# vpc-ccg/freddie

Hardware: AMD Instinct MI355X
Metric: reads segmented/sec (whole node) (higher is better)
Workload: dtype u32

## Files before the change

### freddie_amd/csrc/freddie_seg.hip

```cpp
#include "seg_kernels.h"

using namespace fseg;

namespace {

struct DevBuf {
    void *p = nullptr;
    size_t cap = 0;
    template <typename T> T *as() const { return reinterpret_cast<T *>(p); }
};
struct Slab {
    void *p = nullptr;
    size_t cap = 0;
};
struct HostBuf {
    void *p = nullptr;
    size_t cap = 0;
    template <typename T> T *as() const { return reinterpret_cast<T *>(p); }
};
struct Carve {
    struct Item { DevBuf *b; size_t off, bytes; };
    std::vector<Item> items;
    size_t total = 0;
    size_t add(DevBuf &b, size_t bytes) {
// ... 55 lines not shown
    DevBuf d_packed;
    int fetched_packed = -1;
    bool label_packed_ok = true;
    bool label_has2 = false;
    bool run_label_packed = false;
    bool labels_unpacked = false;
    DevBuf d_sort_tmp;
    DevBuf d_part_iv_off, d_part_rep_off, d_part_lane_off, d_iv_start, d_iv_end, d_pos_off, d_iv_part,
        d_rep_exon_off, d_rep_weight, d_ex_ts, d_ex_te, d_tile_desc, d_iv_tile0, d_blk_iv0, d_rb_part, d_rb_r0, d_rb_sum, d_rb_base, d_rb_max, d_rb_cmax,
        d_hc_part, d_hc_p0, d_hc_n, d_hc_glo, d_hc_ghi;
    DevBuf d_lane_ex, d_lane_start, d_lane_pmax, d_hc_llo, d_hc_lhi, d_key_a, d_key_b, d_val_a, d_val_b, d_rep_last;
    DevBuf d_lane_lx, d_lex, d_rb_esum, d_rb_ebase;
    i64 max_rep_exons = 0;
    DevBuf d_w_main, d_w_refine, d_h_table, d_thr_tab;
    DevBuf d_bits;
    DevBuf d_y_raw, d_y, d_v, d_scan_state, d_bsum, d_bsum_side, d_g, d_pk, d_pf, d_kp;
    int n_hist_chunks = 0;
    DevBuf d_voff, d_chunk_off, d_csum, d_mean, d_thr, d_label_off, d_part_has2;
    int n_rep_blocks = 0;
    DevBuf d_cand_off, d_cand_y, d_fixed0, d_added, d_fixed, d_chosen, d_final_off, d_final_y, d_final_pos, d_final_iv, d_col_thr,
        d_col_zero;
    DevBuf d_tile_defer;
    DevBuf d_blk_pre, d_tile_tot, d_seg_iv, d_seg_prev, d_rseg_c, d_cand_pn, d_cand_ll, d_cand_ln, d_cand_wide, d_prob_bs;
    DevBuf d_prob_iv, d_prob_start, d_prob_n, d_prob_pair_off, d_prob_tri_off, d_prob_flags, d_prob_chain,
        d_prob_cov_off, d_prob_lane_lo, d_prob_lane_n;
    DevBuf d_dp_items, d_solve_items, d_solve_desc, d_prob_desc, d_work_pc, d_cls_items, d_work_active, d_pair_thr, d_amb, d_out, d_cov;
    DevBuf d_wide_items;
    DevBuf d_wide_all;
    DevBuf d_dpx;
    i64 dpx_base[3] = {0, 0, 0}, dpx_stride[3] = {0, 0, 0}, dpx_n[3] = {0, 0, 0};
    int dpx_nm = 0, dpx_cnt[3] = {1, 1, 1};
// ... 298 lines not shown
        if (!dev_sync) return;
        for (int k = 1; k < ps.n_seg; ++k) if (dev_side(k)) (void)fork(ps.side_of[k]);
    };
    auto launch_fork_waiters = [&]() {
        if (!dev_sync) return;
        for (int k = 1; k < ps.n_seg; ++k) if (dev_side(k))
            hipLaunchKernelGGL(k_wait_word, dim3(1), dim3(64), 0, c->side[ps.side_of[k]], st, &sw->emit_gen, 1u, sync_gen, kSyncTicks);
    };
    const i64 avg_len = NPOS / (K > 0 ? K : 1);
    const int iv_threads = avg_len > 65536 ? 1024 : (avg_len > 16384 ? 256 : 64);
    int tile_grid = grid_for(c->n_tiles, 1, 16384);
    const i64 scan_nb = scan_blocks(NPOS);
    const int scan_grid = scan_nb > 0 ? (int)scan_nb : 1;
    u64 *scan_state = c->d_scan_state.as<u64>();
    const bool scan_single = scan_nb <= c->scan_single_max;
    int *bsum = scan_single ? nullptr : c->d_bsum.as<int>();
    int *bsum_side = scan_single ? nullptr : c->d_bsum_side.as<int>();
    auto scan_counts = [&](hipStream_t q, int *bs, const unsigned *flags, u64 *total_dev, i64 *off_last) {
        if (scan_single) return;
        hipLaunchKernelGGL(k_scan1, dim3(grid_for(scan_nb, 1, 4096)), dim3(256), 0, q, flags, NPOS, bs);
        hipLaunchKernelGGL(k_scan2, dim3(1), dim3(kScan2Threads), 0, q, bs, scan_nb, total_dev, off_last);
    };
    int work_grid = grid_for(c->work_cap, 1, 4096);
    ProblemArrays pr{c->d_prob_iv.as<int>(), c->d_prob_start.as<int>(), c->d_prob_n.as<int>(),
                     c->d_prob_pair_off.as<i64>(), c->d_prob_tri_off.as<i64>(), c->d_prob_flags.as<int>(),
                     c->d_prob_chain.as<int>(), c->d_prob_cov_off.as<i64>(), c->d_prob_lane_lo.as<int>(),
                     c->d_prob_lane_n.as<int>()};
    const int pg = grid_for(NPOS / 8 / kProbBlock + 1, 1, 1024);
    i64 *prob_bs = (c->prob_self_scan && !sized) ? nullptr : c->d_prob_bs.as<i64>();
    if (do_pre1) {
    {
        const i64 nw = 3 * (i64)flag_words(NPOS);
// ... 24 lines not shown
#undef FSEG_LAUNCH_SMOOTH
    end(ST_SMOOTH);
    {
    hipStream_t q = fork(0);
    if (stage_events && c->profile_all) (void)hipEventRecord(c->ev_b[ST_THRESHOLD], q);
    const bool thr_part_fits = c->max_part_pos <= (i64)kThrPartMaxChunks * 8192;
    const bool thr_part = thr_part_fits && (c->thr_part == 1 || (c->thr_part < 0 && n_part >= 64));
    if (thr_part) {
        c->paths[fseg_ctx::PATH_THR_PART] = 1;
        hipLaunchKernelGGL(k_thr_part, dim3(grid_for(n_part, 1, 4096)), dim3(512), 0, q, n_part, c->d_part_iv_off.as<i64>(), c->d_pos_off.as<i64>(), NPOS,
                           flag_pos_bits, c->d_y.as<double>(), c->d_v.as<double>(), c->P.variance_factor, c->d_mean.as<double>(), c->d_thr.as<double>());
    } else {
    c->paths[fseg_ctx::PATH_THR_PART] = 0;
    scan_counts(q, bsum_side, flag_pos_bits, &st->n_vals, nullptr);
    hipLaunchKernelGGL(k_scan_emit<kEmitValues>, dim3(scan_grid), dim3(256), 0, q, flag_pos_bits, NPOS,
                       bsum_side, scan_state, &st->n_vals, (i64 *)nullptr, &st->err, c->d_y.as<double>(), c->d_v.as<double>(), K, c->d_pos_off.as<i64>(),
                       c->d_iv_start.as<int>(), c->d_blk_iv0.as<int>(), (int *)nullptr, (int *)nullptr, (i64 *)nullptr,
                       c->force_scan_stall ? 1 : 0, (int *)nullptr);
    hipLaunchKernelGGL(k_voff, dim3(grid_for(n_part + 1, 1, 2048)), dim3(64), 0, q, n_part, c->d_part_iv_off.as<i64>(),
                       c->d_pos_off.as<i64>(), NPOS, flag_pos_bits, bsum_side, scan_state, &st->n_vals,
                       c->d_voff.as<i64>());
    hipLaunchKernelGGL(k_vplan, dim3(1), dim3(256), 0, q, n_part, c->d_part_iv_off.as<i64>(), c->d_pos_off.as<i64>(), NPOS,
                       c->d_voff.as<i64>(), c->d_chunk_off.as<i64>(), st, c->chunk_cap);
    int chunk_grid = grid_for(c->chunk_cap, 1, 4096);
    double *csum0 = c->d_csum.as<double>(), *csum1 = csum0 + c->chunk_cap;
    for (int pass = 0; pass < 2; ++pass)
        hipLaunchKernelGGL(k_vsum_chunks, dim3(chunk_grid), dim3(512), 0, q, n_part, c->d_voff.as<i64>(),
                           c->d_chunk_off.as<i64>(), c->d_v.as<double>(), csum0, pass, pass ? csum1 : csum0, c->chunk_cap);
    hipLaunchKernelGGL(k_vsum_part, dim3(grid_for(n_part, 64, 1024)), dim3(64), 0, q, n_part, c->d_voff.as<i64>(),
                       c->d_chunk_off.as<i64>(), csum0, csum1, c->P.variance_factor, c->d_mean.as<double>(),
                       c->d_thr.as<double>(), c->chunk_cap);
    }
    if (stage_events && c->profile_all) (void)hipEventRecord(c->ev_e[ST_THRESHOLD], q);
    }
    begin(ST_CANDIDATES);
    hipLaunchKernelGGL(k_peaks_edges, dim3(grid_for(c->n_tiles, 256, 4096)), dim3(256), 0, s, c->n_tiles, c->d_tile_desc.as<TileDesc>(),
                       c->d_tile_defer.as<int>(), c->d_y.as<double>(), flag_cand_bits, c->d_part_has2.as<int>(), n_part);
    scan_counts(s, bsum, flag_cand_bits, &st->n_cand, c->d_cand_off.as<i64>() + K);
    hipLaunchKernelGGL(k_scan_emit<kEmitPositions>, dim3(scan_grid), dim3(256), 0, s, flag_cand_bits, NPOS,
                       bsum, scan_state + scan_nb, &st->n_cand, c->d_cand_off.as<i64>() + K, &st->err, (const double *)nullptr, (double *)nullptr, K, c->d_pos_off.as<i64>(),
                       c->d_iv_start.as<int>(), c->d_blk_iv0.as<int>(), c->d_cand_y.as<int>(), (int *)nullptr,
                       c->d_cand_off.as<i64>(), 0, (int *)nullptr);
    end(ST_CANDIDATES);
    join(0);
    early_fork();
    begin(ST_FIX);
    c->paths[fseg_ctx::PATH_IV_THREADS] = iv_threads;
    hipLaunchKernelGGL(k_fix, dim3(grid_for(K, 1, 8192)), dim3(iv_threads), 0, s, K, c->d_pos_off.as<i64>(),
                       c->d_iv_part.as<int>(), c->d_cand_off.as<i64>(), c->d_cand_y.as<int>(), c->d_y.as<double>(),
                       c->d_thr.as<double>(), c->P.max_problem_size, c->d_fixed0.as<unsigned char>(),
                       c->d_added.as<unsigned char>(), c->d_fixed.as<unsigned char>(), c->d_chosen.as<unsigned char>(),
                       c->d_cand_pn.as<int>(), c->d_seg_iv.as<int>(), st);
    i64 *range_bs = prob_bs;
    hipLaunchKernelGGL(k_prob_range, dim3(pg), dim3(kRangeThreads), 0, s, st, c->d_cand_pn.as<int>(),
                       c->d_seg_iv.as<int>(), c->d_cand_y.as<int>(), c->d_iv_part.as<int>(), c->d_iv_start.as<int>(),
// ... 332 lines not shown
                               pr, c->d_prob_desc.as<ProbDesc>(), c->prob_cap, c->d_cand_y.as<int>(), c->d_out.as<unsigned>(),
                               c->tri_cap, c->d_amb.as<unsigned>(), c->d_pair_thr.as<int2>(), c->pair_cap,
                               c->P.min_read_support_outside, c->d_chosen.as<unsigned char>(), c->nm_giant,
                               c->d_giant.as<unsigned char>(), (i64)giant_scratch_bytes(c->nm_giant));
    }
    end(ST_DP); begin(ST_REFINE);
    hipLaunchKernelGGL(k_segments, dim3(grid_for(K, 1, 8192)), dim3(iv_threads), 0, s, K, c->d_pos_off.as<i64>(),
                       c->d_cand_off.as<i64>(), c->d_cand_y.as<int>(), c->d_y_raw.as<int>(), c->d_blk_pre.as<int>(), c->d_tile_tot.as<int>(), c->d_iv_tile0.as<int>(),
                       c->d_chosen.as<unsigned char>(), flag_final_bits, c->d_rseg_c.as<int>(),
                       c->d_seg_prev.as<int>(), st);
    hipLaunchKernelGGL(k_refine, dim3(2048), dim3(64), 0, s, st, c->d_seg_iv.as<int>(), c->d_rseg_c.as<int>(),
                       c->d_seg_prev.as<int>(), c->d_cand_y.as<int>(), c->d_pos_off.as<i64>(), c->d_y_raw.as<int>(),
                       c->d_w_refine.as<double>(), c->P.radius_refine, c->P.sigma, c->d_g.as<double>(), c->d_pk.as<int>(),
                       c->d_pf.as<unsigned char>(), c->d_kp.as<unsigned char>(), flag_final_bits);
    end(ST_REFINE); begin(ST_FINAL);
    scan_counts(s, bsum, flag_final_bits, &st->n_final, c->d_final_off.as<i64>() + K);
    hipLaunchKernelGGL(k_scan_emit<kEmitPositions>, dim3(scan_grid), dim3(256), 0, s, flag_final_bits,
                       NPOS, bsum, scan_state + 2 * scan_nb, &st->n_final, c->d_final_off.as<i64>() + K, &st->err, (const double *)nullptr, (double *)nullptr, K, c->d_pos_off.as<i64>(),
                       c->d_iv_start.as<int>(), c->d_blk_iv0.as<int>(), c->d_final_y.as<int>(), c->d_final_pos.as<int>(),
                       c->d_final_off.as<i64>(), 0, c->d_final_iv.as<int>());
    hipLaunchKernelGGL(k_label_cols, dim3(grid_for(NPOS / 8 + 1, 256, 2048)), dim3(256), 0, s, K, c->d_final_off.as<i64>(),
                       c->d_final_y.as<int>(), c->d_final_iv.as<int>(), c->d_iv_part.as<int>(), c->d_h_table.as<double>(), c->P.h_len,
                       c->P.threshold_rate, c->d_thr_tab.as<int2>(), c->d_col_thr.as<int2>(), c->d_col_zero.as<unsigned char>(),
                       c->d_part_has2.as<int>(), n_part, c->d_part_iv_off.as<i64>(), c->d_part_rep_off.as<i64>(),
                       c->d_label_off.as<i64>(), st, c->label_cap);
    end(ST_FINAL);
    }
    if (do_post2) {
    begin(ST_LABEL);
    if (c->label_cap > 0) {
        c->run_label_packed = lab_packed; c->labels_unpacked = false;
        c->paths[fseg_ctx::PATH_LABEL_PACKED] = lab_packed;
        if (lab_packed) {
// ... 551 lines not shown
        }
    }
    int hist_chunk = hist_packed ? kHistChunk16 : kHistChunk;
    while (hist_chunk > 1024 && NPOS / hist_chunk < 512) hist_chunk >>= 1;
    i64 n_chunks = 0;
    {
        i64 k = 0, pos = 0;
        for (int p = 0; p < np; ++p) {
            i64 Pp = 0;
            for (k = b->part_iv_off[p]; k < b->part_iv_off[p + 1]; ++k) Pp += (i64)b->iv_end[k] - b->iv_start[k] + 1;
            n_chunks += (Pp + hist_chunk - 1) / hist_chunk;
            pos += Pp;
        }
        (void)pos;
    }
    const i64 nb = scan_blocks(NPOS);
    if (n_tiles >= 0x7fffffffLL || n_chunks >= 0x7fffffffLL) return fail(c, FSEG_ERR_UNSUPPORTED, "batch too large");
    Carve in;
    in.add(c->d_part_iv_off, ((size_t)np + 1) * 8);
    in.add(c->d_part_rep_off, ((size_t)np + 1) * 8);
    in.add(c->d_part_lane_off, ((size_t)np + 1) * 8);
    in.add(c->d_iv_start, (size_t)K * 4);
    in.add(c->d_iv_end, (size_t)K * 4);
    in.add(c->d_pos_off, ((size_t)K + 1) * 8);
    in.add(c->d_iv_part, (size_t)K * 4);
    in.add(c->d_iv_tile0, (size_t)K * 4);
    in.add(c->d_tile_desc, (size_t)n_tiles * sizeof(TileDesc));
    in.add(c->d_blk_iv0, ((size_t)nb + 1) * 4);
    in.add(c->d_rb_part, (size_t)n_rep_blocks * 4);
    in.add(c->d_rb_r0, (size_t)n_rep_blocks * 4);
    in.add(c->d_hc_part, (size_t)n_chunks * 4);
    in.add(c->d_hc_p0, (size_t)n_chunks * 8);
    in.add(c->d_hc_n, (size_t)n_chunks * 4);
    in.add(c->d_hc_glo, (size_t)n_chunks * 4);
    in.add(c->d_hc_ghi, (size_t)n_chunks * 4);
    in.add(c->d_rep_exon_off, ((size_t)R + 1) * 8);
    in.add(c->d_rep_weight, (size_t)R * 4);
    in.add(c->d_ex_ts, (size_t)I * 4 + kExonPad);
    in.add(c->d_ex_te, (size_t)I * 4 + kExonPad);
    const size_t up_bytes = in.total;
    in.add(c->d_lane_ex, (size_t)lanes * 16);
    in.add(c->d_lane_start, (size_t)lanes * 4);
    in.add(c->d_lane_pmax, (size_t)lanes * 4);
// ... 25 lines not shown
        int *h_blk = reinterpret_cast<int *>(host_of(c->d_blk_iv0));
        int *h_rb_part = reinterpret_cast<int *>(host_of(c->d_rb_part)), *h_rb_r0 = reinterpret_cast<int *>(host_of(c->d_rb_r0));
        int *h_hc_part = reinterpret_cast<int *>(host_of(c->d_hc_part)), *h_hc_n = reinterpret_cast<int *>(host_of(c->d_hc_n));
        int *h_hc_glo = reinterpret_cast<int *>(host_of(c->d_hc_glo)), *h_hc_ghi = reinterpret_cast<int *>(host_of(c->d_hc_ghi));
        i64 *h_hc_p0 = reinterpret_cast<i64 *>(host_of(c->d_hc_p0));
        h_pos_off[0] = 0; h_lane_off[0] = 0; c->max_part_lanes = 0; c->max_part_pos = 0;
        i64 t = 0, rb = 0, ch = 0, l = 0, bq = 0;
        for (int p = 0; p < np; ++p) {
            const i64 k0 = b->part_iv_off[p], k1 = b->part_iv_off[p + 1];
            for (i64 k = k0; k < k1; ++k) {
                const i64 len = (i64)b->iv_end[k] - b->iv_start[k] + 1;
                h_iv_part[k] = p;
                h_pos_off[k + 1] = h_pos_off[k] + len;
                h_iv_tile0[k] = (int)t;
                for (i64 y = 0; y < len; y += kSmoothTile) h_tile[t++] = TileDesc{h_pos_off[k], (int)y, (int)len};
                for (; bq < nb && bq * kScanBlock < h_pos_off[k + 1]; ++bq) h_blk[bq] = (int)k;
            }
            for (i64 r = b->part_rep_off[p]; r < b->part_rep_off[p + 1]; r += 256) { h_rb_part[rb] = p; h_rb_r0[rb] = (int)r; ++rb; }
            for (i64 r = b->part_rep_off[p]; r < b->part_rep_off[p + 1]; ++r) l += b->rep_weight[r];
            h_lane_off[p + 1] = l;
            if (l - h_lane_off[p] > c->max_part_lanes) c->max_part_lanes = l - h_lane_off[p];
            const i64 P0 = h_pos_off[k0], P1 = h_pos_off[k1];
            if (P1 - P0 > c->max_part_pos) c->max_part_pos = P1 - P0;
            i64 k = k0;
            for (i64 q0 = P0; q0 < P1; q0 += hist_chunk) {
                const i64 q1 = std::min<i64>(q0 + hist_chunk, P1) - 1;
                while (h_pos_off[k + 1] <= q0) ++k;
                i64 kk = k;
                while (h_pos_off[kk + 1] <= q1) ++kk;
                h_hc_part[ch] = p; h_hc_p0[ch] = q0; h_hc_n[ch] = (int)(q1 - q0 + 1);
                h_hc_glo[ch] = b->iv_start[k] + (int)(q0 - h_pos_off[k]);
                h_hc_ghi[ch] = b->iv_start[kk] + (int)(q1 - h_pos_off[kk]);
                ++ch;
            }
        }
        h_blk[nb] = (int)(K - 1);
    }
    const double t_tables = tk.ms();
    memcpy(host_of(c->d_part_iv_off), b->part_iv_off, ((size_t)np + 1) * 8);
    memcpy(host_of(c->d_part_rep_off), b->part_rep_off, ((size_t)np + 1) * 8);
    memcpy(host_of(c->d_iv_start), b->iv_start, (size_t)K * 4);
    memcpy(host_of(c->d_iv_end), b->iv_end, (size_t)K * 4);
    memcpy(host_of(c->d_rep_exon_off), b->rep_exon_off, ((size_t)R + 1) * 8);
    memcpy(host_of(c->d_rep_weight), b->rep_weight, (size_t)R * 4);
    memcpy(host_of(c->d_ex_ts), b->ex_ts, (size_t)I * 4);
    memcpy(host_of(c->d_ex_te), b->ex_te, (size_t)I * 4);
    const double t_copy = tk.ms();
    c->n_part = np; c->K = K; c->R = R; c->I = I; c->NPOS = NPOS; c->LANES = lanes; c->expanded = expanded;
    if (c->max_part_lanes > lanes) c->max_part_lanes = lanes;
    c->n_tiles = (int)n_tiles; c->n_hist_chunks = (int)n_chunks; c->hist_packed = hist_packed; c->n_rep_blocks = (int)n_rep_blocks; c->max_rep_exons = max_rep_exons;
    c->part_iv_off.assign(b->part_iv_off, b->part_iv_off + np + 1);
// ... 46 lines not shown
        }
    }
    hipLaunchKernelGGL(k_hist_ranges, dim3(grid_for(n_chunks, 256, 4096)), dim3(256), 0, s, (int)n_chunks, c->d_hc_part.as<int>(),
                       c->d_hc_glo.as<int>(), c->d_hc_ghi.as<int>(), c->d_part_lane_off.as<i64>(), c->d_lane_start.as<int>(),
                       c->d_lane_pmax.as<int>(), c->d_hc_llo.as<i64>(), c->d_hc_lhi.as<i64>());
    HIP_TRY(c, hipMemcpyAsync(c->h_prep, c->d_prep.p, sizeof(PrepStatus), hipMemcpyDeviceToHost, s));
    HIP_TRY(c, hipGetLastError());
    {
        const size_t np8 = (size_t)NPOS + 64;
        auto atleast = [](i64 &cap, i64 v) { if (cap < v) cap = v; };
        atleast(c->chunk_cap, NPOS / 8192 + np + 8);
        Carve cv;
        cv.add(c->d_y_raw, np8 * 4); cv.add(c->d_y, np8 * 8); cv.add(c->d_bits, 3 * flag_words(np8) * 4);
        cv.add(c->d_v, np8 * 8);
        cv.add(c->d_scan_state, ((size_t)nb * 3 + 1) * 8);
        cv.add(c->d_bsum, ((size_t)nb + 2) * 4);
        cv.add(c->d_bsum_side, ((size_t)nb + 2) * 4);
        cv.add(c->d_g, np8 * 8); cv.add(c->d_pk, np8 * 4); cv.add(c->d_pf, np8); cv.add(c->d_kp, np8);
        cv.add(c->d_part_has2, ((size_t)np + 1) * 4);
        cv.add(c->d_tile_tot, ((size_t)n_tiles + 1) * 4);
        cv.add(c->d_blk_pre, ((size_t)n_tiles + 1) * (kSmoothTile / kSumBlock) * 4);
        cv.add(c->d_tile_defer, ((size_t)n_tiles + 1) * 4);
        cv.add(c->d_voff, ((size_t)np + 2) * 8); cv.add(c->d_chunk_off, ((size_t)np + 2) * 8);
        cv.add(c->d_mean, ((size_t)np + 1) * 8); cv.add(c->d_thr, ((size_t)np + 1) * 8);
        cv.add(c->d_label_off, ((size_t)np + 2) * 8);
        cv.add(c->d_csum, (size_t)c->chunk_cap * 16);
        cv.add(c->d_cand_off, ((size_t)K + 2) * 8); cv.add(c->d_final_off, ((size_t)K + 2) * 8);
        cv.add(c->d_cand_y, np8 * 4); cv.add(c->d_fixed0, np8); cv.add(c->d_added, np8);
        cv.add(c->d_fixed, np8); cv.add(c->d_chosen, np8);
        cv.add(c->d_final_y, np8 * 4); cv.add(c->d_final_pos, np8 * 4); cv.add(c->d_final_iv, np8 * 4); cv.add(c->d_col_thr, np8 * 8); cv.add(c->d_col_zero, np8);
        cv.add(c->d_seg_iv, np8 * 4); cv.add(c->d_seg_prev, np8 * 4); cv.add(c->d_rseg_c, np8 * 4);
// ... 579 lines not shown
```

### freddie_amd/csrc/seg_common.h

```cpp
#pragma once
#include <hip/hip_runtime.h>
#include <type_traits>
#include <hsa/hsa.h>
#include <hsa/hsa_ext_amd.h>
#include <chrono>
#include <algorithm>
#include <atomic>
#include <mutex>
#include <cmath>
#include <cstdarg>
#include <cstdio>
#include <cstdlib>
#include <cstring>
#include <string>
#include <vector>

#include "freddie_seg.h"

namespace fseg {


typedef long long i64;

typedef unsigned long long u64;


constexpr int kSmoothShift = 9;

constexpr int kSmoothTile = 1 << kSmoothShift;

constexpr int kSmoothThreads = kSmoothTile / 4;

constexpr int kSumShift = 4, kSumBlock = 1 << kSumShift;

static_assert(kSmoothTile / kSumBlock <= 64 && kSumBlock == 16, "a tile's block sums are scanned by one wave; a block is four threads' positions");

constexpr int kMaxRadius = 200;

constexpr int kScanBlock = 8192;

inline size_t flag_words(i64 n_pos) { return ((size_t)n_pos + 31) / 32 + 64; }

constexpr int kNMax = 60;

constexpr int kNHuge = 128;

constexpr int kNGiant = 1024;

constexpr int kLaneChunk = 256;

constexpr int kSub = 64;

constexpr i64 kNegInf = (i64)(-0x7fffffffffffffffLL - 1);

// ... 216 lines not shown
    *total = tot;
    return off + x - v;
}


typedef unsigned Flags32;

__device__ __forceinline__ Flags32 load_flags32(const unsigned *flags, i64 i0, i64 n) {
    unsigned w = flags[i0 >> 5];
    if (i0 + 32 > n) w &= n > i0 ? ((1u << (int)(n - i0)) - 1u) : 0u;
    return w;
}

__device__ __forceinline__ int count_flags32(Flags32 f) { return __popc(f); }

__device__ __forceinline__ void set_flag(unsigned *flags, i64 p) { atomicOr(&flags[p >> 5], 1u << (int)(p & 31)); }

constexpr int kScan2Threads = 1024, kScan2Per = 8;

constexpr u64 kScanValueMask = (1ULL << 62) - 1ULL;

__device__ __forceinline__ i64 scan_lookback(u64 *state, i64 b, i64 nb, i64 agg, i64 *bcast , u64 *total_out,
                                             i64 *off_last, unsigned *err) {
    const int lane = lane_id();
    if (threadIdx.x < 64) {
        if (lane == 0)
            __hip_atomic_store(&state[b], ((b == 0 ? 2ULL : 1ULL) << 62) | (u64)agg, __ATOMIC_RELEASE, __HIP_MEMORY_SCOPE_AGENT);
        i64 excl = 0;
        if (b > 0) {
            i64 base = b - 1;
// ... 281 lines not shown
        for (int u = 0; u < 4; ++u) {
            const bool hit0 = eb + 2 * u < n_ex && x[u].y >= cp0 && x[u].x < c_last;
            if (hit0 && cnt == 0) fr = eb + 2 * u;
            cnt += hit0;
            const bool hit1 = eb + 2 * u + 1 < n_ex && x[u].w >= cp0 && x[u].z < c_last;
            if (hit1 && cnt == 0) fr = eb + 2 * u + 1;
            cnt += hit1;
        }
        if (eb + 7 < n_ex && x[3].z >= c_last) break;
    }
    *first_rel = fr; *cnt_out = cnt;
}


constexpr int kRangeThreads = 1024;


constexpr int kProbCols = 9;

__device__ __forceinline__ i64 col_lo(i64 x) { return x & 0xffffffffLL; }

__device__ __forceinline__ i64 col_hi(i64 x) { return (i64)((u64)x >> 32); }

constexpr int kDpSmall = 32;

constexpr int kClsSmall = 16, kClsMid = 32;

struct ProbSizes { i64 v[kProbCols]; };

__device__ __forceinline__ int size_class(int n) { return n <= kClsSmall ? 0 : (n <= kClsMid ? 1 : (n <= kNMax ? 2 : 3)); }
// ... 657 lines not shown
```

### freddie_amd/csrc/seg_front.hip

```cpp
#include "seg_kernels.h"

#include <type_traits>

namespace fseg {

__global__ void __launch_bounds__(256) k_thr_table(const double *h_table, int h_len, double tau, int2 *tab) {
    for (int L = blockIdx.x * blockDim.x + threadIdx.x; L < kThrTab; L += gridDim.x * blockDim.x) {
        int hi = 0x7fffffff, lo = -1;
        if (L >= 1) label_thresholds((i64)L, h_table, h_len, tau, &hi, &lo);
        tab[L] = make_int2(hi, lo);
    }
}

template <int BITS>
__global__ void __launch_bounds__(512) k_hist(int n_chunks, const int *chunk_part, const i64 *chunk_p0, const int *chunk_n,
                                              const int *chunk_glo, const int *chunk_ghi, const i64 *chunk_lane_lo,
                                              const i64 *chunk_lane_hi, const i64 *part_iv_off,
                                              const int *iv_start, const int *iv_end, const i64 *pos_off,
                                              const i64 *part_lane_off, const int2 *__restrict__ lane_lx, const int *lane_start,
                                              const int *lane_pmax, const int2 *__restrict__ lex,
                                              int ignore_ends, int *y_raw, Status *st, u64 *zero_ptr, i64 zero_n) {
    static_assert(BITS == 32 || BITS == 16, "a counter is a word or half a word");
    using Word = std::conditional_t<BITS == 16, unsigned, int>;
    constexpr int kWords = BITS == 16 ? kHistChunk16 / 2 : kHistChunk;
// ... 317 lines not shown
        for (int e = 0; e < kScan2Per; ++e) { v[e] = base + e < nb ? bsum[base + e] : 0; }
#pragma unroll
        for (int e = 0; e < kScan2Per; ++e) { const int x = v[e]; v[e] = run; run += x; }
        int tot;
        const int ex = wg_exclusive_scan<kScan2Threads / 64>(run, lds, &tot);
        const int carry = carry_s;
#pragma unroll
        for (int e = 0; e < kScan2Per; ++e) if (base + e < nb) bsum[base + e] = carry + ex + v[e];
        __syncthreads();
        if (threadIdx.x == 0) carry_s = carry + tot;
        __syncthreads();
    }
    if (threadIdx.x == 0) { *total_out = (u64)carry_s; if (off_last) *off_last = (i64)carry_s; }
}

template <int MODE>
__global__ void __launch_bounds__(256) k_scan_emit(const unsigned *flags, i64 n, const int *bsum ,
                                                   u64 *state, u64 *total_out, i64 *off_last ,
                                                   unsigned *err, const double *y,
                                                   double *v, i64 K, const i64 *pos_off, const int *iv_start,
                                                   const int *blk_iv0, int *out_y, int *out_pos, i64 *out_off,
                                                   int force_stall , int *out_iv ) {
    if (force_stall && !bsum && blockIdx.x == 0 && threadIdx.x == 0) atomicOr(err, kErrScanStall);
    __shared__ int wave_cnt[4];
    __shared__ int lds[16];
    __shared__ i64 bcast;
    const int lane = lane_id(), wave = threadIdx.x >> 6;
    const u64 lt_mask = (1ULL << lane) - 1ULL;
    i64 nb = (n + kScanBlock - 1) / kScanBlock;
    if (MODE == kEmitPositions) {
        constexpr int kIvStage = 768;
        __shared__ i64 po_s[kIvStage + 1];
        __shared__ int is_s[kIvStage];
        {
            const i64 b = blockIdx.x;
            const i64 ka0 = blk_iv0[b], kb0 = (i64)blk_iv0[b + 1] + 1;
            const int niv = (int)(kb0 - ka0);
            const bool staged = niv <= kIvStage;
            if (staged) {
                for (int x = threadIdx.x; x <= niv; x += blockDim.x) po_s[x] = pos_off[ka0 + x];
                for (int x = threadIdx.x; x < niv; x += blockDim.x) is_s[x] = iv_start[ka0 + x];
            }
            i64 i0 = b * kScanBlock + (i64)threadIdx.x * 32;
            Flags32 f = 0;
            int s = 0;
            if (i0 < n) { f = load_flags32(flags, i0, n); s = count_flags32(f); }
            int tot;
            int ex = wg_exclusive_scan<4>(s, lds, &tot);
            ex += bsum ? bsum[b] : (int)scan_lookback(state, b, nb, tot, &bcast, total_out, off_last, err);
            if (s) {
                i64 k = -1, k_end = 0, k_base = 0;
                int k_start = 0;
                {
                    unsigned w = f;
                    while (w) {
                        int e = __ffs(w) - 1;
                        w &= w - 1;
                        i64 i = i0 + e;
                        if (k < 0 || i >= k_end) {
                            const i64 ka = k < 0 ? ka0 : k + 1;
                            if (staged) {
                                const int a = (int)(ka - ka0);
                                const int kk = a + (int)last_le(po_s + a, (i64)(niv - a), i);
                                k = ka0 + kk; k_base = po_s[kk]; k_end = po_s[kk + 1]; k_start = is_s[kk];
                            } else {
                                k = ka + last_le(pos_off + ka, kb0 - ka, i);
                                k_base = pos_off[k]; k_end = pos_off[k + 1]; k_start = iv_start[k];
                            }
                        }
                        int yy = (int)(i - k_base);
                        out_y[ex] = yy;
                        if (out_pos) out_pos[ex] = k_start + yy;
                        if (out_iv) out_iv[ex] = (int)k;
                        if (yy == 0) out_off[k] = ex;
                        ++ex;
                    }
                }
            }
        }
        return;
    }
    {
        const i64 b = blockIdx.x;
        const i64 w0 = b * kScanBlock + (i64)wave * 2048;
        int s = 0;
        unsigned fm = 0;
        {
            i64 i0 = w0 + (i64)lane * 32;
            if (i0 < n) {
                fm = load_flags32(flags, i0, n);
                s = count_flags32(fm);
            }
        }
        for (int d = 32; d >= 1; d >>= 1) s += __shfl_xor(s, d);
        if (lane == 0) wave_cnt[wave] = s;
        __syncthreads();
        const int tot = wave_cnt[0] + wave_cnt[1] + wave_cnt[2] + wave_cnt[3];
        int ex = bsum ? bsum[b] : (int)scan_lookback(state, b, nb, tot, &bcast, total_out, off_last, err);
        for (int w = 0; w < wave; ++w) ex += wave_cnt[w];
        if (s) {
            i64 k = -1, k_end = 0, k_base = 0;
            u64 rows = 0;
            {
                const u64 lanes_set = __ballot(fm != 0);
                u64 pairs = (lanes_set | (lanes_set >> 1)) & 0x5555555555555555ULL;
                pairs = (pairs | (pairs >> 1)) & 0x3333333333333333ULL;
                pairs = (pairs | (pairs >> 2)) & 0x0f0f0f0f0f0f0f0fULL;
                pairs = (pairs | (pairs >> 4)) & 0x00ff00ff00ff00ffULL;
                pairs = (pairs | (pairs >> 8)) & 0x0000ffff0000ffffULL;
                rows = (pairs | (pairs >> 16)) & 0x00000000ffffffffULL;
            }
            while (rows) {
                u64 m[8];
                double yv[8];
                int qs[8];
#pragma unroll
                for (int e = 0; e < 8; ++e) {
                    const int q = rows ? (int)__builtin_ctzll(rows) : -1;
                    qs[e] = q;
                    rows = rows ? rows & (rows - 1) : 0;
                    const int qq = q < 0 ? 0 : q;
                    const unsigned lo = (unsigned)__builtin_amdgcn_readlane((int)fm, 2 * qq);
                    const unsigned hi = (unsigned)__builtin_amdgcn_readlane((int)fm, 2 * qq + 1);
                    m[e] = q < 0 ? 0 : ((u64)lo | ((u64)hi << 32));
                    const i64 i = w0 + qq * 64 + lane;
                    if (MODE == kEmitValues) yv[e] = y[i < n ? i : n - 1];
                }
#pragma unroll
                for (int e = 0; e < 8; ++e) {
                    if (!m[e]) continue;
                    const i64 i = w0 + qs[e] * 64 + lane;
                    if ((m[e] >> lane) & 1ULL) {
                        const int d = ex + __popcll(m[e] & lt_mask);
                        if (MODE == kEmitValues) v[d] = yv[e];
                        else {
                            if (k < 0 || i >= k_end) {
                                const i64 ka = k < 0 ? blk_iv0[b] : k, kb = (i64)blk_iv0[b + 1] + 1;
                                k = ka + last_le(pos_off + ka, kb - ka, i);
                                k_base = pos_off[k]; k_end = pos_off[k + 1];
                            }
                            int yy = (int)(i - k_base);
                            out_y[d] = yy;
                            if (out_pos) out_pos[d] = iv_start[k] + yy;
                            if (out_iv) out_iv[d] = (int)k;
                            if (yy == 0) out_off[k] = d;
                        }
                    }
                    ex += __popcll(m[e]);
                }
            }
        }
    }
}

__global__ void __launch_bounds__(64) k_voff(int n_part, const i64 *part_iv_off, const i64 *pos_off, i64 n_pos,
                                             const unsigned *flags, const int *bsum , const u64 *state, const u64 *total, i64 *voff) {
    for (int p = blockIdx.x; p <= n_part; p += gridDim.x) {
        if (p == n_part) { if (threadIdx.x == 0) voff[p] = (i64)*total; continue; }
        i64 pos = pos_off[part_iv_off[p]];
        i64 b = pos / kScanBlock, start = b * kScanBlock;
        int cnt = 0;
// ... 168 lines not shown
```

### freddie_amd/csrc/seg_kernels.h

```cpp
#pragma once
#include "seg_common.h"

namespace fseg {

__global__ void __launch_bounds__(256) k_thr_table(const double *h_table, int h_len, double tau, int2 *tab);

template <int BITS>
__global__ void __launch_bounds__(512) k_hist(int n_chunks, const int *chunk_part, const i64 *chunk_p0, const int *chunk_n,
                                              const int *chunk_glo, const int *chunk_ghi, const i64 *chunk_lane_lo,
                                              const i64 *chunk_lane_hi, const i64 *part_iv_off,
                                              const int *iv_start, const int *iv_end, const i64 *pos_off,
                                              const i64 *part_lane_off, const int2 *__restrict__ lane_lx, const int *lane_start,
                                              const int *lane_pmax, const int2 *__restrict__ lex,
                                              int ignore_ends, int *y_raw, Status *st, u64 *zero_ptr, i64 zero_n);

template <int R>
#ifndef FSEG_SMOOTH_OCC
#define FSEG_SMOOTH_OCC 6
#endif
__global__ void __launch_bounds__(kSmoothThreads, FSEG_SMOOTH_OCC) k_smooth(int n_tiles, const TileDesc *__restrict__ tiles,
                                                const int *__restrict__ y_raw, const double *__restrict__ w_g, int radius_rt,
                                                double *y_out, unsigned *flag_pos, unsigned *flag_cand, int *blk_pre, int *tile_tot,
                                                int *tile_defer);

__global__ void __launch_bounds__(256) k_clear(Status *st, unsigned *bits, i64 n_words);

__global__ void __launch_bounds__(256) k_scan1(const unsigned *flags, i64 n, int *bsum);

__global__ void __launch_bounds__(kScan2Threads) k_scan2(int *bsum, i64 nb, u64 *total_out, i64 *off_last );

template <int MODE>
__global__ void __launch_bounds__(256) k_scan_emit(const unsigned *flags, i64 n, const int *bsum ,
                                                   u64 *state, u64 *total_out, i64 *off_last ,
                                                   unsigned *err, const double *y,
                                                   double *v, i64 K, const i64 *pos_off, const int *iv_start,
                                                   const int *blk_iv0, int *out_y, int *out_pos, i64 *out_off,
                                                   int force_stall , int *out_iv );

__global__ void __launch_bounds__(64) k_voff(int n_part, const i64 *part_iv_off, const i64 *pos_off, i64 n_pos,
                                             const unsigned *flags, const int *bsum , const u64 *state, const u64 *total, i64 *voff);

__global__ void __launch_bounds__(256) k_vplan(int n_part, const i64 *part_iv_off, const i64 *pos_off, i64 n_pos,
                                               i64 *voff, i64 *chunk_off, Status *st, i64 chunk_cap);

__global__ void __launch_bounds__(512) k_vsum_chunks(int n_part, const i64 *voff, const i64 *chunk_off, const double *v,
                                                     const double *csum0, int pass, double *csum, i64 chunk_cap);

__global__ void __launch_bounds__(512) k_thr_part(int n_part, const i64 *part_iv_off, const i64 *pos_off, i64 n_pos, const unsigned *flags,
// ... 221 lines not shown
```

### freddie_amd/csrc/seg_problems.hip

```cpp
#include "seg_kernels.h"

namespace fseg {


__global__ void k_fix(i64 K, const i64 *pos_off, const int *iv_part, const i64 *cand_off, const int *cand_y,
                      const double *yv, const double *thr_part, int mps, unsigned char *fixed0, unsigned char *added,
                      unsigned char *fixed, unsigned char *chosen, int *cand_pn, int *cand_iv, Status *st) {
    __shared__ int lds[16];
    const int T = blockDim.x;
    for (i64 k = blockIdx.x; k < K; k += gridDim.x) {
        i64 c0 = cand_off[k];
        int N = (int)(cand_off[k + 1] - c0);
        const double *y = yv + pos_off[k];
        const int *cy = cand_y + c0;
        double thr = thr_part[iv_part[k]];
        if (T == 64 && N <= 64 && N <= mps) {
            const int c = threadIdx.x;
            const bool in = c < N;
            const bool f = in && (c == 0 || c == N - 1 || y[cy[c]] > thr);
            const u64 mask = __ballot(f);
            int n = 0;
            if (in) {
                const u64 below = mask & ((1ULL << c) - 1ULL);
                const int prev = below ? 63 - __clzll((long long)below) : -1;
// ... 51 lines not shown
            }
        }
        __syncthreads();
    }
}

__global__ void __launch_bounds__(kRangeThreads) k_prob_range(Status *st, const int *cand_pn, const int *cand_iv, const int *cand_y,
                             const int *iv_part, const int *iv_start, const i64 *part_lane_off, const int *lane_start,
                             const int *lane_pmax, int *cand_ll, int *cand_ln, unsigned char *cand_wide,
                             const int2 *__restrict__ lane_lx, const int2 *__restrict__ lex, int wide_by_seen, int fuse_lanes,
                             i64 *bs, ProbSplit sp) {
    static_assert(kRangeThreads == kProbBlock, "a workgroup of k_prob_range is a block of the problem scan");
    __shared__ int l_wide[kRangeThreads], l_n, l_red[kRangeThreads / 64];
    __shared__ i64 scan_lds[4 * kProbCols];
    __shared__ int l_mx[8];
    const i64 n_cand = (i64)st->n_cand;
    for (i64 c0 = (i64)blockIdx.x * blockDim.x; c0 < n_cand; c0 += (i64)gridDim.x * blockDim.x) {
        const i64 c = c0 + threadIdx.x;
        if (threadIdx.x == 0) l_n = 0;
        __syncthreads();
        if (c < n_cand) {
            int n = cand_pn[c];
            int lo_lane = 0, n_lanes = 0;
            if (n > 0) {
                int k = cand_iv[c];
                int part = iv_part[k];
                int g0 = iv_start[k] + cand_y[c - (n - 1)], g1 = iv_start[k] + cand_y[c];
                i64 a = part_lane_off[part], L1 = part_lane_off[part + 1], b = L1;
                while (a < b) { i64 m = (a + b) >> 1; if (lane_pmax[m] < g0) a = m + 1; else b = m; }
                i64 lo = a;
                b = L1;
                while (a < b) { i64 m = (a + b) >> 1; if (lane_start[m] < g1) a = m + 1; else b = m; }
                lo_lane = (int)lo; n_lanes = (int)(a - lo);
            }
            cand_ll[c] = lo_lane; cand_ln[c] = n_lanes;
            const bool cand = n > 0 && n <= kNMax && n_lanes > kFuseLanes && n_lanes <= kFuseLanesWide && n_lanes <= fuse_lanes;
            cand_wide[c] = (unsigned char)((cand && wide_by_seen) ? 1 : 0);
            if (cand && !wide_by_seen) l_wide[atomicAdd(&l_n, 1)] = (int)threadIdx.x;
        }
        __syncthreads();
        const int nw = l_n;
        for (int w = 0; w < nw; ++w) {
            const i64 cw = c0 + l_wide[w];
            const int n = cand_pn[cw], k = cand_iv[cw], ll = cand_ll[cw], ln = cand_ln[cw];
            const int cp0 = iv_start[k] + cand_y[cw - (n - 1)], c_last = iv_start[k] + cand_y[cw];
            int kept = 0;
            for (int l = threadIdx.x; l < ln; l += kRangeThreads) {
                int first_rel, cnt;
// ... 223 lines not shown
```

Measured before the change: 591.0 million.

## Use larger position-scan blocks with two-level count and stage lane tables in LDS

Position-mode scan-emit now runs on 32K-position blocks with 128-bit flag loads. A new k_pos_count kernel produces per-block and per-group sums, and each block builds its prefix from those sums, replacing the k_scan1/k_scan2 pair for candidates and finals. The value-mode emit path drops its dead position branch. Separately, k_prob_range stages the workgroup's lane_pmax/lane_start range into LDS so its binary searches read shared memory instead of global. This trades fewer, larger blocks and fewer launches for more work per thread and extra LDS use, which may lower occupancy.

```diff
diff --git a/freddie_amd/csrc/freddie_seg.hip b/freddie_amd/csrc/freddie_seg.hip
--- a/freddie_amd/csrc/freddie_seg.hip
+++ b/freddie_amd/csrc/freddie_seg.hip
@@ -93,7 +93,7 @@
     i64 max_rep_exons = 0;
     DevBuf d_w_main, d_w_refine, d_h_table, d_thr_tab;
     DevBuf d_bits;
-    DevBuf d_y_raw, d_y, d_v, d_scan_state, d_bsum, d_bsum_side, d_g, d_pk, d_pf, d_kp;
+    DevBuf d_y_raw, d_y, d_v, d_scan_state, d_bsum, d_gsum, d_bsum_side, d_g, d_pk, d_pf, d_kp;
     int n_hist_chunks = 0;
     DevBuf d_voff, d_chunk_off, d_csum, d_mean, d_thr, d_label_off, d_part_has2;
     int n_rep_blocks = 0;
@@ -422,8 +422,16 @@
     const int scan_grid = scan_nb > 0 ? (int)scan_nb : 1;
     u64 *scan_state = c->d_scan_state.as<u64>();
     const bool scan_single = scan_nb <= c->scan_single_max;
-    int *bsum = scan_single ? nullptr : c->d_bsum.as<int>();
     int *bsum_side = scan_single ? nullptr : c->d_bsum_side.as<int>();
+    const i64 pos_nb = pos_blocks(NPOS);
+    const int pos_grid = pos_nb > 0 ? (int)pos_nb : 1;
+    const bool pos_single = scan_single;
+    int *bsum = pos_single ? nullptr : c->d_bsum.as<int>();
+    int *gsum = pos_single ? nullptr : c->d_gsum.as<int>();
+    auto pos_counts = [&](hipStream_t q, const unsigned *flags) {
+        if (pos_single) return;
+        hipLaunchKernelGGL(k_pos_count, dim3(grid_for(pos_groups(NPOS), 1, 4096)), dim3(kPosCountThreads), 0, q, flags, NPOS, bsum, gsum);
+    };
     auto scan_counts = [&](hipStream_t q, int *bs, const unsigned *flags, u64 *total_dev, i64 *off_last) {
         if (scan_single) return;
         hipLaunchKernelGGL(k_scan1, dim3(grid_for(scan_nb, 1, 4096)), dim3(256), 0, q, flags, NPOS, bs);
@@ -478,7 +486,7 @@
     c->paths[fseg_ctx::PATH_THR_PART] = 0;
     scan_counts(q, bsum_side, flag_pos_bits, &st->n_vals, nullptr);
     hipLaunchKernelGGL(k_scan_emit<kEmitValues>, dim3(scan_grid), dim3(256), 0, q, flag_pos_bits, NPOS,
-                       bsum_side, scan_state, &st->n_vals, (i64 *)nullptr, &st->err, c->d_y.as<double>(), c->d_v.as<double>(), K, c->d_pos_off.as<i64>(),
+                       bsum_side, (const int *)nullptr, scan_state, &st->n_vals, (i64 *)nullptr, &st->err, c->d_y.as<double>(), c->d_v.as<double>(), K, c->d_pos_off.as<i64>(),
                        c->d_iv_start.as<int>(), c->d_blk_iv0.as<int>(), (int *)nullptr, (int *)nullptr, (i64 *)nullptr,
                        c->force_scan_stall ? 1 : 0, (int *)nullptr);
     hipLaunchKernelGGL(k_voff, dim3(grid_for(n_part + 1, 1, 2048)), dim3(64), 0, q, n_part, c->d_part_iv_off.as<i64>(),
@@ -500,9 +508,9 @@
     begin(ST_CANDIDATES);
     hipLaunchKernelGGL(k_peaks_edges, dim3(grid_for(c->n_tiles, 256, 4096)), dim3(256), 0, s, c->n_tiles, c->d_tile_desc.as<TileDesc>(),
                        c->d_tile_defer.as<int>(), c->d_y.as<double>(), flag_cand_bits, c->d_part_has2.as<int>(), n_part);
-    scan_counts(s, bsum, flag_cand_bits, &st->n_cand, c->d_cand_off.as<i64>() + K);
-    hipLaunchKernelGGL(k_scan_emit<kEmitPositions>, dim3(scan_grid), dim3(256), 0, s, flag_cand_bits, NPOS,
-                       bsum, scan_state + scan_nb, &st->n_cand, c->d_cand_off.as<i64>() + K, &st->err, (const double *)nullptr, (double *)nullptr, K, c->d_pos_off.as<i64>(),
+    pos_counts(s, flag_cand_bits);
+    hipLaunchKernelGGL(k_scan_emit<kEmitPositions>, dim3(pos_grid), dim3(256), 0, s, flag_cand_bits, NPOS,
+                       bsum, gsum, scan_state + scan_nb, &st->n_cand, c->d_cand_off.as<i64>() + K, &st->err, (const double *)nullptr, (double *)nullptr, K, c->d_pos_off.as<i64>(),
                        c->d_iv_start.as<int>(), c->d_blk_iv0.as<int>(), c->d_cand_y.as<int>(), (int *)nullptr,
                        c->d_cand_off.as<i64>(), 0, (int *)nullptr);
     end(ST_CANDIDATES);
@@ -865,9 +873,9 @@
                        c->d_w_refine.as<double>(), c->P.radius_refine, c->P.sigma, c->d_g.as<double>(), c->d_pk.as<int>(),
                        c->d_pf.as<unsigned char>(), c->d_kp.as<unsigned char>(), flag_final_bits);
     end(ST_REFINE); begin(ST_FINAL);
-    scan_counts(s, bsum, flag_final_bits, &st->n_final, c->d_final_off.as<i64>() + K);
-    hipLaunchKernelGGL(k_scan_emit<kEmitPositions>, dim3(scan_grid), dim3(256), 0, s, flag_final_bits,
-                       NPOS, bsum, scan_state + 2 * scan_nb, &st->n_final, c->d_final_off.as<i64>() + K, &st->err, (const double *)nullptr, (double *)nullptr, K, c->d_pos_off.as<i64>(),
+    pos_counts(s, flag_final_bits);
+    hipLaunchKernelGGL(k_scan_emit<kEmitPositions>, dim3(pos_grid), dim3(256), 0, s, flag_final_bits,
+                       NPOS, bsum, gsum, scan_state + 2 * scan_nb, &st->n_final, c->d_final_off.as<i64>() + K, &st->err, (const double *)nullptr, (double *)nullptr, K, c->d_pos_off.as<i64>(),
                        c->d_iv_start.as<int>(), c->d_blk_iv0.as<int>(), c->d_final_y.as<int>(), c->d_final_pos.as<int>(),
                        c->d_final_off.as<i64>(), 0, c->d_final_iv.as<int>());
     hipLaunchKernelGGL(k_label_cols, dim3(grid_for(NPOS / 8 + 1, 256, 2048)), dim3(256), 0, s, K, c->d_final_off.as<i64>(),
@@ -1449,7 +1457,7 @@
         }
         (void)pos;
     }
-    const i64 nb = scan_blocks(NPOS);
+    const i64 nb = scan_blocks(NPOS), nbp = pos_blocks(NPOS);
     if (n_tiles >= 0x7fffffffLL || n_chunks >= 0x7fffffffLL) return fail(c, FSEG_ERR_UNSUPPORTED, "batch too large");
     Carve in;
     in.add(c->d_part_iv_off, ((size_t)np + 1) * 8);
@@ -1461,7 +1469,7 @@
     in.add(c->d_iv_part, (size_t)K * 4);
     in.add(c->d_iv_tile0, (size_t)K * 4);
     in.add(c->d_tile_desc, (size_t)n_tiles * sizeof(TileDesc));
-    in.add(c->d_blk_iv0, ((size_t)nb + 1) * 4);
+    in.add(c->d_blk_iv0, ((size_t)nbp + 1) * 4);
     in.add(c->d_rb_part, (size_t)n_rep_blocks * 4);
     in.add(c->d_rb_r0, (size_t)n_rep_blocks * 4);
     in.add(c->d_hc_part, (size_t)n_chunks * 4);
@@ -1517,7 +1525,7 @@
                 h_pos_off[k + 1] = h_pos_off[k] + len;
                 h_iv_tile0[k] = (int)t;
                 for (i64 y = 0; y < len; y += kSmoothTile) h_tile[t++] = TileDesc{h_pos_off[k], (int)y, (int)len};
-                for (; bq < nb && bq * kScanBlock < h_pos_off[k + 1]; ++bq) h_blk[bq] = (int)k;
+                for (; bq < nbp && bq * kPosBlock < h_pos_off[k + 1]; ++bq) h_blk[bq] = (int)k;
             }
             for (i64 r = b->part_rep_off[p]; r < b->part_rep_off[p + 1]; r += 256) { h_rb_part[rb] = p; h_rb_r0[rb] = (int)r; ++rb; }
             for (i64 r = b->part_rep_off[p]; r < b->part_rep_off[p + 1]; ++r) l += b->rep_weight[r];
@@ -1537,7 +1545,7 @@
                 ++ch;
             }
         }
-        h_blk[nb] = (int)(K - 1);
+        h_blk[nbp] = (int)(K - 1);
     }
     const double t_tables = tk.ms();
     memcpy(host_of(c->d_part_iv_off), b->part_iv_off, ((size_t)np + 1) * 8);
@@ -1614,7 +1622,8 @@
         cv.add(c->d_y_raw, np8 * 4); cv.add(c->d_y, np8 * 8); cv.add(c->d_bits, 3 * flag_words(np8) * 4);
         cv.add(c->d_v, np8 * 8);
         cv.add(c->d_scan_state, ((size_t)nb * 3 + 1) * 8);
-        cv.add(c->d_bsum, ((size_t)nb + 2) * 4);
+        cv.add(c->d_bsum, ((size_t)nbp + 2) * 4);
+        cv.add(c->d_gsum, ((size_t)pos_groups(NPOS) + 2) * 4);
         cv.add(c->d_bsum_side, ((size_t)nb + 2) * 4);
         cv.add(c->d_g, np8 * 8); cv.add(c->d_pk, np8 * 4); cv.add(c->d_pf, np8); cv.add(c->d_kp, np8);
         cv.add(c->d_part_has2, ((size_t)np + 1) * 4);
diff --git a/freddie_amd/csrc/seg_common.h b/freddie_amd/csrc/seg_common.h
--- a/freddie_amd/csrc/seg_common.h
+++ b/freddie_amd/csrc/seg_common.h
@@ -38,6 +38,14 @@
 constexpr int kMaxRadius = 200;
 
 constexpr int kScanBlock = 8192;
+
+constexpr int kPosBlock = 32768;
+constexpr int kPosGroup = 64;
+constexpr int kPosCountThreads = 1024;
+static_assert(kPosBlock % (64 * 128) == 0 && kPosGroup % (kPosCountThreads / 64) == 0 && kPosGroup <= 64,
+              "k_pos_count: a wave takes whole blocks, 64 lanes x 16 bytes a round; k_scan_emit: a wave adds a group's block sums in one round");
+inline i64 pos_blocks(i64 n) { return (n + kPosBlock - 1) / kPosBlock; }
+inline i64 pos_groups(i64 n) { return (pos_blocks(n) + kPosGroup - 1) / kPosGroup; }
 
 inline size_t flag_words(i64 n_pos) { return ((size_t)n_pos + 31) / 32 + 64; }
 
@@ -284,6 +292,19 @@
 
 __device__ __forceinline__ int count_flags32(Flags32 f) { return __popc(f); }
 
+__device__ __forceinline__ void load_flags128(const unsigned *flags, i64 i0, i64 n, Flags32 w[4]) {
+    const int4u v = *reinterpret_cast<const int4u *>(flags + (i0 >> 5));
+    w[0] = (unsigned)v.x; w[1] = (unsigned)v.y; w[2] = (unsigned)v.z; w[3] = (unsigned)v.w;
+    if (i0 + 128 > n) {
+#pragma unroll
+        for (int j = 0; j < 4; ++j) {
+            const i64 left = n - (i0 + 32 * j);
+            if (left < 32) w[j] &= left > 0 ? ((1u << (int)left) - 1u) : 0u;
+        }
+    }
+}
+__device__ __forceinline__ int count_flags128(const Flags32 w[4]) { return __popc(w[0]) + __popc(w[1]) + __popc(w[2]) + __popc(w[3]); }
+
 __device__ __forceinline__ void set_flag(unsigned *flags, i64 p) { atomicOr(&flags[p >> 5], 1u << (int)(p & 31)); }
 
 constexpr int kScan2Threads = 1024, kScan2Per = 8;
@@ -595,6 +616,7 @@
 
 
 constexpr int kRangeThreads = 1024;
+constexpr int kRangeStage = 4096;
 
 
 constexpr int kProbCols = 9;
diff --git a/freddie_amd/csrc/seg_front.hip b/freddie_amd/csrc/seg_front.hip
--- a/freddie_amd/csrc/seg_front.hip
+++ b/freddie_amd/csrc/seg_front.hip
@@ -355,9 +355,47 @@
     if (threadIdx.x == 0) { *total_out = (u64)carry_s; if (off_last) *off_last = (i64)carry_s; }
 }
 
+__global__ void __launch_bounds__(kPosCountThreads) k_pos_count(const unsigned *flags, i64 n, int *bsum, int *gsum) {
+    __shared__ int wsum[kPosCountThreads / 64];
+    constexpr int kPer = kPosGroup / (kPosCountThreads / 64);
+    const int lane = lane_id(), wave = threadIdx.x >> 6;
+    const i64 nb = (n + kPosBlock - 1) / kPosBlock;
+    for (i64 g = blockIdx.x; g * kPosGroup < nb; g += gridDim.x) {
+        int cnt[kPer];
+#pragma unroll
+        for (int j = 0; j < kPer; ++j) {
+            const i64 b = g * kPosGroup + wave * kPer + j;
+            int s = 0;
+#pragma unroll
+            for (int r = 0; r < kPosBlock / (64 * 128); ++r) {
+                const i64 i0 = b * kPosBlock + (i64)(r * 64 + lane) * 128;
+                if (i0 < n) { Flags32 f[4]; load_flags128(flags, i0, n, f); s += count_flags128(f); }
+            }
+            cnt[j] = s;
+        }
+        int tot = 0;
+#pragma unroll
+        for (int j = 0; j < kPer; ++j) {
+            int x = cnt[j];
+            for (int d = 32; d >= 1; d >>= 1) x += __shfl_xor(x, d);
+            const i64 b = g * kPosGroup + wave * kPer + j;
+            if (lane == 0 && b < nb) bsum[b] = x;
+            tot += x;
+        }
+        if (lane == 0) wsum[wave] = tot;
+        __syncthreads();
+        if (threadIdx.x == 0) {
+            int t = 0;
+            for (int w = 0; w < kPosCountThreads / 64; ++w) t += wsum[w];
+            gsum[g] = t;
+        }
+        __syncthreads();
+    }
+}
+
 template <int MODE>
 __global__ void __launch_bounds__(256) k_scan_emit(const unsigned *flags, i64 n, const int *bsum ,
-                                                   u64 *state, u64 *total_out, i64 *off_last ,
+                                                   const int *gsum , u64 *state, u64 *total_out, i64 *off_last ,
                                                    unsigned *err, const double *y,
                                                    double *v, i64 K, const i64 *pos_off, const int *iv_start,
                                                    const int *blk_iv0, int *out_y, int *out_pos, i64 *out_off,
@@ -368,13 +406,14 @@
     __shared__ i64 bcast;
     const int lane = lane_id(), wave = threadIdx.x >> 6;
     const u64 lt_mask = (1ULL << lane) - 1ULL;
-    i64 nb = (n + kScanBlock - 1) / kScanBlock;
     if (MODE == kEmitPositions) {
         constexpr int kIvStage = 768;
         __shared__ i64 po_s[kIvStage + 1];
         __shared__ int is_s[kIvStage];
+        __shared__ int pre_s;
         {
             const i64 b = blockIdx.x;
+            const i64 nbp = (n + kPosBlock - 1) / kPosBlock;
             const i64 ka0 = blk_iv0[b], kb0 = (i64)blk_iv0[b + 1] + 1;
             const int niv = (int)(kb0 - ka0);
             const bool staged = niv <= kIvStage;
@@ -382,22 +421,38 @@
                 for (int x = threadIdx.x; x <= niv; x += blockDim.x) po_s[x] = pos_off[ka0 + x];
                 for (int x = threadIdx.x; x < niv; x += blockDim.x) is_s[x] = iv_start[ka0 + x];
             }
-            i64 i0 = b * kScanBlock + (i64)threadIdx.x * 32;
-            Flags32 f = 0;
+            if (bsum && wave == 0) {
+                int p = 0;
+                const i64 g = b / kPosGroup;
+                for (i64 j = lane; j < g; j += 64) p += gsum[j];
+                for (i64 j = g * kPosGroup + lane; j < b; j += 64) p += bsum[j];
+                for (int d = 32; d >= 1; d >>= 1) p += __shfl_xor(p, d);
+                if (lane == 0) pre_s = p;
+            }
+            const i64 i0 = b * kPosBlock + (i64)threadIdx.x * 128;
+            Flags32 f[4] = {0u, 0u, 0u, 0u};
             int s = 0;
-            if (i0 < n) { f = load_flags32(flags, i0, n); s = count_flags32(f); }
+            if (i0 < n) { load_flags128(flags, i0, n, f); s = count_flags128(f); }
             int tot;
             int ex = wg_exclusive_scan<4>(s, lds, &tot);
-            ex += bsum ? bsum[b] : (int)scan_lookback(state, b, nb, tot, &bcast, total_out, off_last, err);
+            if (bsum) {
+                const int pre = pre_s;
+                ex += pre;
+                if (b == nbp - 1 && threadIdx.x == 0) {
+                    *total_out = (u64)((i64)pre + tot);
+                    if (off_last) *off_last = (i64)pre + tot;
+                }
+            } else ex += (int)scan_lookback(state, b, nbp, tot, &bcast, total_out, off_last, err);
             if (s) {
                 i64 k = -1, k_end = 0, k_base = 0;
                 int k_start = 0;
-                {
-                    unsigned w = f;
+#pragma unroll
+                for (int j = 0; j < 4; ++j) {
+                    unsigned w = f[j];
                     while (w) {
                         int e = __ffs(w) - 1;
                         w &= w - 1;
-                        i64 i = i0 + e;
+                        i64 i = i0 + 32 * j + e;
                         if (k < 0 || i >= k_end) {
                             const i64 ka = k < 0 ? ka0 : k + 1;
                             if (staged) {
@@ -422,7 +477,7 @@
         return;
     }
     {
-        const i64 b = blockIdx.x;
+        const i64 b = blockIdx.x, nb = (n + kScanBlock - 1) / kScanBlock;
         const i64 w0 = b * kScanBlock + (i64)wave * 2048;
         int s = 0;
         unsigned fm = 0;
@@ -440,7 +495,6 @@
         int ex = bsum ? bsum[b] : (int)scan_lookback(state, b, nb, tot, &bcast, total_out, off_last, err);
         for (int w = 0; w < wave; ++w) ex += wave_cnt[w];
         if (s) {
-            i64 k = -1, k_end = 0, k_base = 0;
             u64 rows = 0;
             {
                 const u64 lanes_set = __ballot(fm != 0);
@@ -454,38 +508,23 @@
             while (rows) {
                 u64 m[8];
                 double yv[8];
-                int qs[8];
 #pragma unroll
                 for (int e = 0; e < 8; ++e) {
                     const int q = rows ? (int)__builtin_ctzll(rows) : -1;
-                    qs[e] = q;
                     rows = rows ? rows & (rows - 1) : 0;
                     const int qq = q < 0 ? 0 : q;
                     const unsigned lo = (unsigned)__builtin_amdgcn_readlane((int)fm, 2 * qq);
                     const unsigned hi = (unsigned)__builtin_amdgcn_readlane((int)fm, 2 * qq + 1);
                     m[e] = q < 0 ? 0 : ((u64)lo | ((u64)hi << 32));
                     const i64 i = w0 + qq * 64 + lane;
-                    if (MODE == kEmitValues) yv[e] = y[i < n ? i : n - 1];
+                    yv[e] = y[i < n ? i : n - 1];
                 }
 #pragma unroll
                 for (int e = 0; e < 8; ++e) {
                     if (!m[e]) continue;
-                    const i64 i = w0 + qs[e] * 64 + lane;
                     if ((m[e] >> lane) & 1ULL) {
                         const int d = ex + __popcll(m[e] & lt_mask);
-                        if (MODE == kEmitValues) v[d] = yv[e];
-                        else {
-                            if (k < 0 || i >= k_end) {
-                                const i64 ka = k < 0 ? blk_iv0[b] : k, kb = (i64)blk_iv0[b + 1] + 1;
-                                k = ka + last_le(pos_off + ka, kb - ka, i);
-                                k_base = pos_off[k]; k_end = pos_off[k + 1];
-                            }
-                            int yy = (int)(i - k_base);
-                            out_y[d] = yy;
-                            if (out_pos) out_pos[d] = iv_start[k] + yy;
-                            if (out_iv) out_iv[d] = (int)k;
-                            if (yy == 0) out_off[k] = d;
-                        }
+                        v[d] = yv[e];
                     }
                     ex += __popcll(m[e]);
                 }
diff --git a/freddie_amd/csrc/seg_kernels.h b/freddie_amd/csrc/seg_kernels.h
--- a/freddie_amd/csrc/seg_kernels.h
+++ b/freddie_amd/csrc/seg_kernels.h
@@ -29,9 +29,11 @@
 
 __global__ void __launch_bounds__(kScan2Threads) k_scan2(int *bsum, i64 nb, u64 *total_out, i64 *off_last );
 
+__global__ void __launch_bounds__(kPosCountThreads) k_pos_count(const unsigned *flags, i64 n, int *bsum, int *gsum);
+
 template <int MODE>
 __global__ void __launch_bounds__(256) k_scan_emit(const unsigned *flags, i64 n, const int *bsum ,
-                                                   u64 *state, u64 *total_out, i64 *off_last ,
+                                                   const int *gsum , u64 *state, u64 *total_out, i64 *off_last ,
                                                    unsigned *err, const double *y,
                                                    double *v, i64 K, const i64 *pos_off, const int *iv_start,
                                                    const int *blk_iv0, int *out_y, int *out_pos, i64 *out_off,
diff --git a/freddie_amd/csrc/seg_problems.hip b/freddie_amd/csrc/seg_problems.hip
--- a/freddie_amd/csrc/seg_problems.hip
+++ b/freddie_amd/csrc/seg_problems.hip
@@ -89,24 +89,50 @@
     __shared__ int l_wide[kRangeThreads], l_n, l_red[kRangeThreads / 64];
     __shared__ i64 scan_lds[4 * kProbCols];
     __shared__ int l_mx[8];
+    __shared__ int s_pmax[kRangeStage], s_start[kRangeStage];
+    __shared__ i64 l_lane_a, l_lane_b;
     const i64 n_cand = (i64)st->n_cand;
     for (i64 c0 = (i64)blockIdx.x * blockDim.x; c0 < n_cand; c0 += (i64)gridDim.x * blockDim.x) {
         const i64 c = c0 + threadIdx.x;
         if (threadIdx.x == 0) l_n = 0;
-        __syncthreads();
+        int n = 0, g0 = 0, g1 = 0;
+        i64 pa = 0, pb = 0;
         if (c < n_cand) {
-            int n = cand_pn[c];
+            n = cand_pn[c];
+            const int k = cand_iv[c], y1 = cand_y[c];
+            const int part = iv_part[k], is = iv_start[k];
+            const int y0 = cand_y[n > 0 ? c - (n - 1) : c];
+            pa = part_lane_off[part]; pb = part_lane_off[part + 1];
+            g0 = is + y0; g1 = is + y1;
+            if (threadIdx.x == 0) l_lane_a = pa;
+            if (c == n_cand - 1 || threadIdx.x == kRangeThreads - 1) l_lane_b = pb;
+        }
+        __syncthreads();
+        const i64 A = l_lane_a;
+        const int n_stage = (int)(l_lane_b - A < (i64)kRangeStage + 1 ? l_lane_b - A : (i64)kRangeStage + 1);
+        const bool staged = n_stage <= kRangeStage;
+        if (staged) {
+            for (int x = threadIdx.x; x < n_stage; x += kRangeThreads) { s_pmax[x] = lane_pmax[A + x]; s_start[x] = lane_start[A + x]; }
+            __syncthreads();
+        }
+        if (c < n_cand) {
             int lo_lane = 0, n_lanes = 0;
             if (n > 0) {
-                int k = cand_iv[c];
-                int part = iv_part[k];
-                int g0 = iv_start[k] + cand_y[c - (n - 1)], g1 = iv_start[k] + cand_y[c];
-                i64 a = part_lane_off[part], L1 = part_lane_off[part + 1], b = L1;
-                while (a < b) { i64 m = (a + b) >> 1; if (lane_pmax[m] < g0) a = m + 1; else b = m; }
-                i64 lo = a;
-                b = L1;
-                while (a < b) { i64 m = (a + b) >> 1; if (lane_start[m] < g1) a = m + 1; else b = m; }
-                lo_lane = (int)lo; n_lanes = (int)(a - lo);
+                i64 a = pa, L1 = pb, b = L1;
+                if (staged) {
+                    int x = (int)(a - A), xe = (int)(L1 - A), y = xe;
+                    while (x < y) { const int m = (x + y) >> 1; if (s_pmax[m] < g0) x = m + 1; else y = m; }
+                    const int lo = x;
+                    y = xe;
+                    while (x < y) { const int m = (x + y) >> 1; if (s_start[m] < g1) x = m + 1; else y = m; }
+                    lo_lane = (int)(A + lo); n_lanes = x - lo;
+                } else {
+                    while (a < b) { i64 m = (a + b) >> 1; if (lane_pmax[m] < g0) a = m + 1; else b = m; }
+                    i64 lo = a;
+                    b = L1;
+                    while (a < b) { i64 m = (a + b) >> 1; if (lane_start[m] < g1) a = m + 1; else b = m; }
+                    lo_lane = (int)lo; n_lanes = (int)(a - lo);
+                }
             }
             cand_ll[c] = lo_lane; cand_ln[c] = n_lanes;
             const bool cand = n > 0 && n <= kNMax && n_lanes > kFuseLanes && n_lanes <= kFuseLanesWide && n_lanes <= fuse_lanes;
```

Result: faster. 602.6 million (median of 6 runs) (+2.0%).
